# askerlee/segtran

Measured on AMD Instinct MI355X. Metric: train-step images/sec (cfg2, re-associated op order), higher is better.
Workload: dtype f32; 1 GPU; REFUGE fundus 2D, segtran eff-b4, translayers 3, layercompress 1,1,2,2, 512x512, bs 6/GPU; global_batch=6, per_gpu_batch=6, parallelism=dp1, step=fwd+BCE/Dice+bwd+allreduce+clip+BertAdam, op_order=re-associated, ranks=1

## Files before the change

### include/segx.h

```cpp
#ifndef SEGX_H
#define SEGX_H
#include <stdint.h>
#ifdef __cplusplus
extern "C" {
#endif

int segx_version(void);
int segx_last_error(char* buf, int buflen);

enum { SEGX_EPI_NONE = 0, SEGX_EPI_GELU = 1 ,
       SEGX_EPI_SWISH = 2 ,
       SEGX_EPI_RELU = 3  };
enum { SEGX_BIAS_NONE = 0, SEGX_BIAS_N = 1 , SEGX_BIAS_M = 2  };
enum { SEGX_ENGINE_F32 = 0, SEGX_ENGINE_BF16X6 = 1 };
enum { SEGX_ENGINE_SEL_DEFAULT = 0, SEGX_ENGINE_SEL_F32 = 1, SEGX_ENGINE_SEL_BF16X6 = 2 };
enum { SEGX_TILE_AUTO = 0, SEGX_TILE_128x128 = 1, SEGX_TILE_64x64 = 2, SEGX_TILE_128x32 = 3, SEGX_TILE_32x128 = 4, SEGX_TILE_64x128 = 5,
       SEGX_TILE_256x128 = 6, SEGX_TILE_WS128x128 = 7, SEGX_TILE_WS128x256 = 8, SEGX_TILE_WS64x256 = 9,
       SEGX_TILE_WS96x256 = 10, SEGX_TILE_WS256x96 = 11,
       SEGX_TILE_SKINNY_NT = 12   };
typedef struct {
    int32_t M, N, K, nb0, nb1;
    int64_t a_b0, a_b1, a_m, a_k;
    int64_t b_b0, b_b1, b_n, b_k;
    int64_t c_b0, c_b1, c_m;
// ... 102 lines not shown
int segx_team_status(int clear);
int segx_team_cap(void);
int segx_occupy(int wgs, int heavy, float ms, float* sink, void* stream);
int segx_bn_act_bwd2(const float* dY, const float* X, const float* mean, const float* var, const float* w, const float* b,
                     float* dX, float* dw, float* db, float* ws, int B, int C, int64_t S, float eps, int act, int training,
                     const float* gate, const float* dpool, float inv_S, float dc_p, uint64_t seed, uint64_t offset, int64_t dy_bs, int64_t ws_floats, void* stream);
int segx_se_fwd2(const float* psum, int nch, float inv_S, const float* W1, const float* b1, const float* W2, const float* b2, const float* Wproj,
                 float* p, float* hpre, float* gate, float* Wb, int B, int C, int Cs, int M, void* stream);
int64_t segx_se_ws2_floats(int B, int C, int Cs);
int segx_se_bwd2(const float* dWb, const float* Wproj, const float* dgate, const float* gate, const float* hpre, const float* p, const float* W1,
                 const float* W2, float inv_S, float* dpool, float* dW1, float* db1, float* dW2, float* db2, float* dWproj, float* ws,
                 int B, int C, int Cs, int M, void* stream);
int segx_dwconv2d_fwd(const float* X, const float* W, float* Y, int B, int C, int H, int Wd, int OH, int OW, int k, int stride,
                      int pad_t, int pad_l, void* stream);
int64_t segx_dwconv2d_pool_chunks(int OH, int OW);
int segx_dwconv2d_bias_act_pool(const float* X, const float* W, const float* bias, float* Y, float* psum, int B, int C, int H, int Wd, int OH, int OW,
                                int k, int stride, int pad_t, int pad_l, int act, void* stream);
int segx_dwconv2d_bwd_data(const float* dY, const float* W, float* dX, int B, int C, int H, int Wd, int OH, int OW, int k,
                           int stride, int pad_t, int pad_l, void* stream);
int64_t segx_dwconv2d_wgrad_rows(int OH, int OW);
int64_t segx_dwconv2d_bwd_fused_rows(int H, int Wd, int OH, int OW, int k, int stride, int pad_t, int pad_l);
int segx_dwconv2d_bwd_fused(const float* dY, const float* X, const float* W, float* dX, float* part, int B, int C, int H, int Wd, int OH, int OW,
                            int k, int stride, int pad_t, int pad_l, void* stream);
int segx_dwconv2d_bwd_weight_direct(const float* dY, const float* X, float* dW, int B, int C, int H, int Wd, int OH, int OW, int k,
                                    int stride, int pad_t, int pad_l, void* stream);
int segx_dwconv2d_bwd_weight(const float* dY, const float* X, float* part, int B, int C, int H, int Wd, int OH, int OW, int k,
                             int stride, int pad_t, int pad_l, void* stream);
int segx_plane_scale(const float* X, const float* gate, float* Y, int64_t planes, int64_t S, void* stream);
int segx_plane_bias_add(const float* X, const float* bias, float* Y, int64_t planes, int C, int64_t S, void* stream);
int segx_plane_dot(const float* A, const float* Bm, float* out, int64_t planes, int64_t S, void* stream);

int64_t segx_gn_ws_floats(int B, int C, int G);
int segx_groupnorm_fwd(const float* X, const float* w, const float* b, float* Y, float* mean, float* rstd, float* ws,
                       int B, int C, int G, int64_t S, float eps, void* stream);
int segx_groupnorm_bwd(const float* dY, const float* X, const float* w, const float* mean, const float* rstd, float* dX,
                       float* dw, float* db, float* ws, int B, int C, int G, int64_t S, float* plane_dx_sums, void* stream);
int64_t segx_interp_gn_nparts(int64_t float4_per_plane, int cpg);
int segx_interp_linear_fwd_axis2_gn(const float* in, const float* base, float* out, int64_t outer, int n1_in, int n1_out, int n2_in, int n2_out,
                                    int64_t inner, int cpg, float* parts, int nparts, void* stream);
int segx_groupnorm_fwd_parts(const float* X, const float* parts, int nparts, const float* w, const float* b, float* Y, float* mean, float* rstd,
                             int B, int C, int G, int64_t S, float eps, void* stream);
int segx_groupnorm_stats_parts(const float* parts, int nparts, float* mean, float* rstd, int BG, float eps, void* stream);
int segx_gn_fold_bwd_proj(const float* dOut, const float* Wb, int NC, const float* X, const float* mean, const float* rstd, const float* A, const float* Bc,
                          float* dX, float* plane_sums, float* ws, int B, int C, int G, int64_t S, void* stream);
int segx_gn_fold_bwd(const float* Gd, const float* X, const float* mean, const float* rstd, const float* A, const float* Bc, float* dX, float* plane_sums,
                     float* ws, int B, int C, int G, int64_t S, void* stream);
// ... 130 lines not shown
```

### segtran_amd/csrc/backbone.hip

```cpp
#include "common.h"
#include <mutex>
#include <unordered_map>

namespace segx {

enum { ACT_NONE = 0, ACT_SWISH = 1, ACT_RELU = 2, ACT_LEAKY = 3  };

__device__ __forceinline__ float sigm(float x) { return 1.0f / (1.0f + __expf(-x)); }
__device__ __forceinline__ float act_fwd(float u, int act) {
    return act == ACT_SWISH ? u * sigm(u) : act == ACT_RELU ? fmaxf(u, 0.f) : act == ACT_LEAKY ? (u > 0.f ? u : 0.2f * u) : u;
}
__device__ __forceinline__ float act_grad(float u, int act) {
    if (act == ACT_SWISH) { const float s = sigm(u); return s * (1.0f + u * (1.0f - s)); }
    if (act == ACT_RELU) return u > 0.f ? 1.0f : 0.f;
    if (act == ACT_LEAKY) return u > 0.f ? 1.0f : 0.2f;
    return 1.0f;
}

__device__ __forceinline__ float drop_connect_scale(float p, uint64_t seed, uint64_t offset, const uint64_t* __restrict__ rbase, int sample) {
    if (!(p > 0.f)) return 1.0f;
    return dropout_scale(seed, 0, offset + (rbase ? *rbase : 0) + (uint64_t)sample, p, 1.0f / (1.0f - p));
}
__device__ __forceinline__ void bn_fold_sums(const float* __restrict__ ws, int c, int nparts, float& a, float& q) {
    const int lane = threadIdx.x & 63;
    const float2* p = reinterpret_cast<const float2*>(ws) + (int64_t)c * nparts;
    a = 0.f; q = 0.f;
    for (int i = lane; i < nparts; i += 64) { const float2 v = p[i]; a += v.x; q += v.y; }
    a = wave_sum(a); q = wave_sum(q);
}

constexpr int BN_SLABS = 8;
static inline int bn_slabs(int64_t S) { const int64_t n = S / 8192; return (int)(n < 1 ? 1 : n > BN_SLABS ? BN_SLABS : n); }

__global__ __launch_bounds__(256) void bn_act_bwd_stage1(const float* __restrict__ dY, const float* __restrict__ X, const float* __restrict__ mean,
                                                         const float* __restrict__ var, const float* __restrict__ w, const float* __restrict__ b,
                                                         float* __restrict__ ws, int C, int64_t S, float eps, int act,
                                                         const float* __restrict__ gate, const float* __restrict__ dpool, float inv_S,
                                                         float dc_p, uint64_t seed, uint64_t offset, const uint64_t* __restrict__ rbase, int64_t dy_bs) {
    __shared__ float red[4];
    const int c = blockIdx.x, bb = blockIdx.y, slab = blockIdx.z;
// ... 1742 lines not shown
```

### segtran_amd/csrc/common.h

```cpp
#pragma once
#include <hip/hip_runtime.h>
#include <stdint.h>
#include <stdio.h>
#include <stdarg.h>
#include <string.h>
#include <math.h>
#include <atomic>
#include "../../include/segx.h"

typedef float f32x16 __attribute__((ext_vector_type(16)));
typedef float f32x4 __attribute__((ext_vector_type(4)));

namespace segx {

inline char* err_buf() { static thread_local char buf[512] = {0}; return buf; }
inline int fail(int code, const char* fmt, ...) {
    va_list ap; va_start(ap, fmt); vsnprintf(err_buf(), 512, fmt, ap); va_end(ap); return code;
}
inline int check_launch(const char* what) {
    hipError_t e = hipGetLastError();
    if (e != hipSuccess) return fail((int)e, "%s: %s", what, hipGetErrorString(e));
    return 0;
}
#ifndef SEGX_MIN_WAVES_PER_SIMD
// ... 115 lines not shown
    return v;
}
template <int NW> __device__ __forceinline__ float block_sum(float v, float* red) {
    v = wave_sum(v);
    const int lane = threadIdx.x & 63, w = threadIdx.x >> 6;
    __syncthreads();
    if (lane == 0) red[w] = v;
    __syncthreads();
    float s = 0.f;
#pragma unroll
    for (int i = 0; i < NW; ++i) s += red[i];
    return s;
}
template <int NW> __device__ __forceinline__ float block_max(float v, float* red) {
    v = wave_max(v);
    const int lane = threadIdx.x & 63, w = threadIdx.x >> 6;
    __syncthreads();
    if (lane == 0) red[w] = v;
    __syncthreads();
    float s = red[0];
#pragma unroll
    for (int i = 1; i < NW; ++i) s = fmaxf(s, red[i]);
    return s;
}

struct u32x4 { unsigned x, y, z, w; };
__device__ __forceinline__ u32x4 philox4(uint64_t seed, uint64_t ctr) {
    unsigned c0 = (unsigned)ctr, c1 = (unsigned)(ctr >> 32), c2 = 0x5eed5eedu, c3 = 0u;
    unsigned k0 = (unsigned)seed, k1 = (unsigned)(seed >> 32);
#pragma unroll
    for (int r = 0; r < 7; ++r) {
        const unsigned h0 = __umulhi(0xD2511F53u, c0), l0 = 0xD2511F53u * c0;
        const unsigned h1 = __umulhi(0xCD9E8D57u, c2), l1 = 0xCD9E8D57u * c2;
        const unsigned n0 = h1 ^ c1 ^ k0, n2 = h0 ^ c3 ^ k1;
        c0 = n0; c1 = l1; c2 = n2; c3 = l0;
        k0 += 0x9E3779B9u; k1 += 0xBB67AE85u;
    }
    u32x4 o; o.x = c0; o.y = c1; o.z = c2; o.w = c3; return o;
}
__device__ __forceinline__ float keep_of(unsigned u, float p, float inv_keep) {
    return ((float)(u >> 8) * (1.0f / 16777216.0f) >= p) ? inv_keep : 0.0f;
}
__device__ __forceinline__ float4 dropout_scale4(uint64_t seed, uint64_t offset, uint64_t idx0, float p, float inv_keep) {
    const u32x4 r = philox4(seed, (offset + idx0) >> 2);
    return make_float4(keep_of(r.x, p, inv_keep), keep_of(r.y, p, inv_keep), keep_of(r.z, p, inv_keep), keep_of(r.w, p, inv_keep));
}
// ... 82 lines not shown
```

### segtran_amd/efficientnet/model.py

```python
import math
import torch
from torch import nn
from torch.nn import functional as F

from .. import functional as SF

BN_MOM, BN_EPS = 1 - 0.99, 1e-3

_BASE = [(1, 3, 1, 1, 32, 16, 0.25), (2, 3, 2, 6, 16, 24, 0.25), (2, 5, 2, 6, 24, 40, 0.25), (3, 3, 2, 6, 40, 80, 0.25),
         (3, 5, 1, 6, 80, 112, 0.25), (4, 5, 2, 6, 112, 192, 0.25), (1, 3, 1, 6, 192, 320, 0.25)]
_PARAMS = {'efficientnet-b0': (1.0, 1.0, 224, 0.2), 'efficientnet-b1': (1.0, 1.1, 240, 0.2),
           'efficientnet-b2': (1.1, 1.2, 260, 0.3), 'efficientnet-b3': (1.2, 1.4, 300, 0.3),
           'efficientnet-b4': (1.4, 1.8, 380, 0.4), 'efficientnet-b5': (1.6, 2.2, 456, 0.4),
           'efficientnet-b6': (1.8, 2.6, 528, 0.5), 'efficientnet-b7': (2.0, 3.1, 600, 0.5)}


def round_filters(filters, width, divisor=8):
    filters *= width
    new = max(divisor, int(filters + divisor / 2) // divisor * divisor)
    if new < 0.9 * filters:
        new += divisor
    return int(new)


# ... 40 lines not shown
        s = bn.weight.double() / torch.sqrt(bn.running_var.double() + bn.eps)
        w = (weight.double() * s.view(-1, *([1] * (weight.dim() - 1)))).float().contiguous()
        b = (bn.bias.double() - bn.running_mean.double() * s).float().contiguous()
    return w, b


class MBConvBlock(nn.Module):
    def __init__(self, k, s, e, cin, cout, se_ratio, image_size):
        super().__init__()
        self.stride, self.expand_ratio, self.input_filters, self.output_filters = s, e, cin, cout
        oup = cin * e
        if e != 1:
            self._expand_conv = Conv2dStaticSamePadding(cin, oup, 1, image_size=image_size, bias=False)
            self._bn0 = nn.BatchNorm2d(oup, momentum=BN_MOM, eps=BN_EPS)
        self._depthwise_conv = Conv2dStaticSamePadding(oup, oup, k, stride=s, image_size=image_size, groups=oup, bias=False)
        self._bn1 = nn.BatchNorm2d(oup, momentum=BN_MOM, eps=BN_EPS)
        nsq = max(1, int(cin * se_ratio))
        self._se_reduce = Conv2dStaticSamePadding(oup, nsq, 1, image_size=1)
        self._se_expand = Conv2dStaticSamePadding(nsq, oup, 1, image_size=1)
        self._project_conv = Conv2dStaticSamePadding(oup, cout, 1, image_size=math.ceil(image_size / s), bias=False)
        self._bn2 = nn.BatchNorm2d(cout, momentum=BN_MOM, eps=BN_EPS)

    gate_in_weights = True

    def folded_operands(self):
        f0 = fold_conv_bn(self._expand_conv.weight, self._bn0) if self.expand_ratio != 1 else None
        return f0, fold_conv_bn(self._depthwise_conv.weight, self._bn1), fold_conv_bn(self._project_conv.weight, self._bn2)

    def forward_folded(self, inputs, folded):
        f0, (w1, b1), (w2, b2) = folded
        x = inputs
        skip = self.stride == 1 and self.input_filters == self.output_filters
        if f0 is not None:
            x = SF.conv1x1(x, f0[0], f0[1], act=SF.ACT_SWISH)
        dw = self._depthwise_conv
        y, psum, nch = SF.dwconv2d_bias_act_pool(x, w1, b1, dw.stride[0], dw.static_pad, SF.ACT_SWISH)
        Wb = SF.se_gate_weights(y, psum, nch, self._se_reduce.weight, self._se_reduce.bias, self._se_expand.weight, self._se_expand.bias, w2)
        return SF.conv1x1_per_sample_bias(y, Wb, b2, resid=inputs if skip else None)

    def forward(self, inputs, drop_connect_rate=None):
        x = skip_in = inputs
        skip = self.stride == 1 and self.input_filters == self.output_filters
        if self.expand_ratio != 1:
            x = SF.bn_act(self._expand_conv(x), self._bn0, SF.ACT_SWISH)
        se = (self._se_reduce.weight, self._se_reduce.bias, self._se_expand.weight, self._se_expand.bias)
        rate = float(drop_connect_rate) if (skip and drop_connect_rate and self.training) else 0.0
        if MBConvBlock.gate_in_weights:
            y, Wb = SF.bn_act_gate_weights(self._depthwise_conv(x), self._bn1, SF.ACT_SWISH, *se, self._project_conv.weight)
            x = SF.conv1x1_per_sample(y, Wb)
        else:
            x = self._project_conv(SF.bn_act_se(self._depthwise_conv(x), self._bn1, SF.ACT_SWISH, *se))
        return SF.bn_act(x, self._bn2, SF.ACT_NONE, resid=skip_in if skip else None, drop_connect=rate)


class EfficientNet(nn.Module):
    def __init__(self, model_name='efficientnet-b4', stem_stride=2, drop_connect_rate=0.2, num_classes=1000):
        super().__init__()
        width, depth, res, _ = _PARAMS[model_name]
        self.drop_connect_rate = drop_connect_rate
        self.stem_stride = stem_stride
        c0 = round_filters(32, width)
        self._conv_stem = Conv2dStaticSamePadding(3, c0, 3, stride=stem_stride, image_size=res, bias=False)
        self._bn0 = nn.BatchNorm2d(c0, momentum=BN_MOM, eps=BN_EPS)
        size = math.ceil(res / 2)
        self._blocks = nn.ModuleList([])
        self.endpoint_seg_indices = [0, 1, 2, 4]
        self.endpoint_blk_indices = []
        for i, (r, k, s, e, cin, cout, se) in enumerate(_BASE):
            cin, cout, r = round_filters(cin, width), round_filters(cout, width), round_repeats(r, depth)
            self._blocks.append(MBConvBlock(k, s, e, cin, cout, se, size))
# ... 127 lines not shown
```

### segtran_amd/functional.py

```python
import math
import torch
import torch.nn.functional as F
from . import segx
from .segx import EPI_NONE, EPI_GELU, EPI_SWISH, EPI_RELU, BIAS_NONE, BIAS_N, BIAS_M

LN_EPS = 1e-12


_MRO = torch.autograd.Function.__mro__
_fast_apply = torch._C._FunctionBase in _MRO and not any('apply' in c.__dict__ for c in _MRO[1:_MRO.index(torch._C._FunctionBase)])


class _Fn(torch.autograd.Function):

    @classmethod
    def apply(cls, *args):
        if _fast_apply and not torch._C._are_functorch_transforms_active():
            return super(torch.autograd.Function, cls).apply(*args)
        return super().apply(*args)


def _live(t):
    return t.requires_grad and torch.is_grad_enabled()

# ... 974 lines not shown
        ctx.cfg = (B, C, S, eps, act, training, n)
        ctx.shapes = (tuple(w1.shape), tuple(w2.shape), tuple(Wproj.shape))
        ctx.save_for_backward(x, mean, var, w, b, p, hpre, gate, W1, W2, Wp)
        return y, Wb

    @staticmethod
    def backward(ctx, dy, dWb):
        L = segx.lib()
        x, mean, var, w, b, p, hpre, gate, W1, W2, Wp = ctx.saved_tensors
        S = ctx.cfg[2]
        w1s, w2s, wps = ctx.shapes
        dWb = _c(dWb) if dWb is not None else torch.zeros(gate.shape[0], Wp.shape[0], Wp.shape[1], dtype=torch.float32, device=x.device)
        dpool, dW1, db1, dW2, db2, dWp = _se_excite_backward(L, x, dWb, Wp, None, gate, hpre, p, W1, W2, S)
        dx, dw, db = _bn_act_backward(L, _c(dy), x, mean, var, w, b, ctx.cfg, None, dpool, 1.0)
        return dx, dw, db, None, None, None, None, None, None, dW1.view(w1s), db1, dW2.view(w2s), db2, dWp.view(wps)


def bn_act_gate_weights(x, bn, act, w1, b1, w2, b2, proj_weight):
    _bn_tick(bn)
    return _BNActGateW.apply(x, bn.weight, bn.bias, bn.running_mean, bn.running_var, bn.training, float(bn.momentum), float(bn.eps), act, w1, b1, w2, b2,
                             proj_weight)


def conv1x1_per_sample(x, Wb, bias=None):
    B, Cin = x.shape[0], x.shape[1]
    S = x.numel() // (B * Cin)
    Cout = Wb.shape[1]
    if bias is None:
        spec = GemmSpec(Cout, S, Cin, (Cout * Cin, 0, Cin, 1), (Cin * S, 0, 1, S), (Cout * S, 0, S), (B, Cout) + tuple(x.shape[2:]), nb=(B, 1))
        return bgemm(Wb, x, spec)
    spec = GemmSpec(Cout, S, Cin, (Cout * Cin, 0, Cin, 1), (Cin * S, 0, 1, S), (Cout * S, 0, S), (B, Cout) + tuple(x.shape[2:]), nb=(B, 1), bias_mode=BIAS_M, bias_b0=Cout)
    return bgemm(Wb, x, spec, bias=_c(bias))


def dwconv2d_bias_act_pool(x, w, bias, stride, pad, act=ACT_SWISH, pool=True):
    if act not in (ACT_NONE, ACT_SWISH):
        raise NotImplementedError('dwconv2d_bias_act_pool: act is ACT_NONE or ACT_SWISH')
    _no_grad_operands('dwconv2d_bias_act_pool', x, w, bias)
    L = segx.lib()
    x, w = _c(x), _c(w)
    B, C, H, W = x.shape
    k, stride = w.shape[-1], int(stride)
    pl, pr, pt, pb = (int(v) for v in pad)
    OH, OW = (H + pt + pb - k) // stride + 1, (W + pl + pr - k) // stride + 1
    y = _empty(x, B, C, OH, OW)
    nch = L.dwconv2d_pool_chunks(OH, OW) if pool else 0
# ... 1225 lines not shown
```

### segtran_amd/segx.py

```python
import contextlib
import ctypes
import enum
import os
import torch

_HERE = os.path.dirname(os.path.abspath(__file__))
LIB_PATH = os.path.join(_HERE, 'lib', 'libsegx.so')

c_f = ctypes.c_float
c_i = ctypes.c_int32
c_l = ctypes.c_int64
c_u = ctypes.c_uint64
c_p = ctypes.c_void_p


class GemmDesc(ctypes.Structure):
    _fields_ = [('M', c_i), ('N', c_i), ('K', c_i), ('nb0', c_i), ('nb1', c_i),
                ('a_b0', c_l), ('a_b1', c_l), ('a_m', c_l), ('a_k', c_l),
                ('b_b0', c_l), ('b_b1', c_l), ('b_n', c_l), ('b_k', c_l),
                ('c_b0', c_l), ('c_b1', c_l), ('c_m', c_l),
                ('alpha', c_f), ('epilogue', c_i), ('bias_mode', c_i), ('bias_b1', c_l),
                ('bias', c_p), ('aux', c_p), ('gmax', c_p),
                ('dropout_p', c_f), ('seed', c_u), ('offset', c_u),
                ('splitk', c_i), ('workspace', c_p), ('tile', c_i), ('bias_b0', c_l), ('batch_reduce', c_i), ('engine', c_i),
# ... 325 lines not shown
            self._chk_t(Y)
            assert Y.device == X.device and Y.dtype == torch.float32 and Y.stride(1) == S and Y.stride(0) == y_bs and Y[0].is_contiguous()
            Y = Y.data_ptr()
        self._call('segx_bn_act_fwd2', X, X, parts, nparts, mean, var, run_mean, run_var, momentum, w, b, Y, psum, resid, float(dc_p), seed, offset, B, C, S, eps, act,
                   0 if parts is None else parts.numel(), int(y_bs))

    def bn_act_bwd2(self, dY, X, mean, var, w, b, dX, dw, db, ws, B, C, S, eps, act, training, gate=None, dpool=None, inv_S=0.0, dc_p=0.0, seed=0, offset=0, dy_bs=0):
        self._chk_t(dY, X, mean, var, w, b, dX, dw, db, ws, gate, dpool)
        for t in (X, mean, var, w, b, dX, dw, db, ws):
            assert t.is_contiguous()
        assert dy_bs or dY.is_contiguous()
        rc = self.c.segx_bn_act_bwd2(_ptr(dY), _ptr(X), _ptr(mean), _ptr(var), _ptr(w), _ptr(b), _ptr(dX), _ptr(dw), _ptr(db), _ptr(ws), B, C, S, eps, act, training,
                                     _ptr(gate), _ptr(dpool), float(inv_S), float(dc_p), seed, offset, int(dy_bs), ws.numel(), self.stream(X))
        self.check(rc, 'segx_bn_act_bwd2')

    def se_fwd2(self, psum, nch, inv_S, W1, b1, W2, b2, Wproj, p, hpre, gate, Wb, B, C, Cs, M):
        self._call('segx_se_fwd2', gate, psum, nch, inv_S, W1, b1, W2, b2, Wproj, p, hpre, gate, Wb, B, C, Cs, M)

    def se_ws2(self, B, C, Cs):
        return int(self.c.segx_se_ws2_floats(B, C, Cs))

    def se_bwd2(self, dWb, Wproj, dgate, gate, hpre, p, W1, W2, inv_S, dpool, dW1, db1, dW2, db2, dWproj, ws, B, C, Cs, M):
        self._call('segx_se_bwd2', gate, dWb, Wproj, dgate, gate, hpre, p, W1, W2, inv_S, dpool, dW1, db1, dW2, db2, dWproj, ws, B, C, Cs, M)

    def dwconv2d_fwd(self, X, W, Y, B, C, H, Wd, OH, OW, k, stride, pt, pl):
        self._call('segx_dwconv2d_fwd', X, X, W, Y, B, C, H, Wd, OH, OW, k, stride, pt, pl)

    def dwconv2d_pool_chunks(self, OH, OW):
        return int(self.c.segx_dwconv2d_pool_chunks(OH, OW))

    def dwconv2d_bias_act_pool(self, X, W, bias, Y, psum, B, C, H, Wd, OH, OW, k, stride, pt, pl, act):
        self._call('segx_dwconv2d_bias_act_pool', X, X, W, bias, Y, psum, B, C, H, Wd, OH, OW, k, stride, pt, pl, act)

    def dwconv2d_bwd_data(self, dY, W, dX, B, C, H, Wd, OH, OW, k, stride, pt, pl):
        self._call('segx_dwconv2d_bwd_data', dY, dY, W, dX, B, C, H, Wd, OH, OW, k, stride, pt, pl)

    def dwconv2d_bwd_weight_direct(self, dY, X, dW, B, C, H, Wd, OH, OW, k, stride, pt, pl):
        self._chk_t(dY, X, dW)
        rc = self.c.segx_dwconv2d_bwd_weight_direct(_ptr(dY), _ptr(X), _ptr(dW), B, C, H, Wd, OH, OW, k, stride, pt, pl, self.stream(X))
        if rc < 0:
            self.check(rc, 'segx_dwconv2d_bwd_weight_direct')
        return rc == 1

    def dwconv2d_bwd_fused_rows(self, H, W, OH, OW, k, stride, pad_t, pad_l):
        return int(self.c.segx_dwconv2d_bwd_fused_rows(H, W, OH, OW, k, stride, pad_t, pad_l))

# ... 346 lines not shown
    'segx_mt_bertadam_step': 'pppppppppppiiifffddfpp', 'segx_mt_gather': 'pppppiiip',
    'segx_gn_ws_floats': 'iii', 'segx_groupnorm_fwd': 'pppppppiiilfp', 'segx_groupnorm_bwd': 'pppppppppiiilpp',
    'segx_interp_gn_nparts': 'li', 'segx_interp_linear_fwd_axis2_gn': 'pppliiiilipip', 'segx_groupnorm_fwd_parts': 'ppipppppiiilfp',
    'segx_groupnorm_stats_parts': 'pippifp', 'segx_gn_fold_bwd': 'pppppppppiiilp', 'segx_bridge_mask': 'ppppiiiiiiiiip', 'segx_gn_fold_bwd_proj': 'ppippppppppiiilp',
    'segx_interp_linear_fwd': 'pppliiiiiip', 'segx_interp_linear_fwd_axis2': 'pppliiiilp', 'segx_interp_linear_bwd_axis2': 'ppliiiilp', 'segx_interp_linear_bwd': 'ppliiiiiip', 'segx_interp_linear_bwd_axis': 'ppliilfp',
    'segx_axis_gather': 'pplpp', 'segx_pixel_shuffle2': 'ppliiip', 'segx_add_noise': 'ppplffiuup', 'segx_resize2d': 'ppliiiiiip', 'segx_color_blend': 'ppilippip',
    'segx_gray_mean_ws_floats': 'il', 'segx_gray_mean': 'pppilip', 'segx_normalize': 'ppiilfppp',
    'segx_x6_presplit_elems': 'iiii', 'segx_x6_presplit': 'piilliillpp',
    'segx_tune': 'ii', 'segx_tune_get': 'i', 'segx_x3_launches': '', 'segx_gemm_route': 'pppp', 'segx_set_rng_base': 'p', 'segx_rng_advance': 'pup', 'segx_resized_crop3d': 'pplpp', 'segx_stem_compose_fwd': 'ppppiiiiip', 'segx_stem_compose_bwd': 'pppppppiiiiip', 'segx_bridge_input': 'ppiiiiiip', 'segx_stem_s2d_input': 'ppiiiiiip', 'segx_conv2d_stem_fwd': 'pppiiiiiiiiiiip', 'segx_conv2d_stem_im2col': 'ppiiiiiiiiiiip', 'segx_dropout': 'pplfuup', 'segx_avgpool2_fwd': 'ppliip', 'segx_avgpool2_bwd': 'ppliip', 'segx_transpose': 'ppliip', 'segx_interp_linear_fwd_axis': 'pppliilfp', 'segx_window_accum': 'pppiipp', 'segx_harden_segmap': 'ppppiilifp', 'segx_window_gather': 'ppppiiipp', 'segx_window_merge': 'pppppiiipifp', 'segx_dice_ws_floats': 'll', 'segx_dice_sums': 'pppllp',
    'segx_surface_border': 'ppliiiip', 'segx_edt_sq': 'ppliiip', 'segx_surface_hist': 'pppliiiip',
    'segx_ccl2d': 'pippliip', 'segx_frag_keep2': 'ppliip', 'segx_frag_apply': 'ppppliiip', 'segx_row_extent': 'ppliifp', 'segx_nhot_to_values': 'ppplilp',
    'segx_conv3d_fwd': 'pppiipipp', 'segx_conv3d_fwd_packed': 'pppiipipp', 'segx_conv3d_fwd_packed_bs': 'pppiipipllp', 'segx_conv3d_bwd_weight_packed_bs': 'pppiipipllp', 'segx_conv3d_pack_weights': 'ppiiiip', 'segx_conv3d_splitk': 'iipi', 'segx_conv3d_route': 'iipiiiip', 'segx_conv3d_fwd_terms': 'iipiii', 'segx_conv3d_flip_weights': 'ppiiip', 'segx_conv3d_bwd_weight': 'pppiipipp', 'segx_conv3d_bwd_weight_packed': 'pppiipipp', 'segx_conv3d_unpack_wgrad': 'ppiiip',
    'segx_conv3d_halo_ok': 'iip', 'segx_conv3d_halo_wq_floats': 'ii', 'segx_conv3d_halo_pack': 'ppiiip', 'segx_conv3d_halo_fwd': 'pppiipllip', 'segx_conv3d_halo_bias_act_fwd': 'ppppiiplliip', 'segx_conv3d_fwd_bias_act': 'ppppiipipillip', 'segx_bias_map_relu': 'ppilp', 'segx_conv3d_halo_wgrad_ok': 'iip', 'segx_conv3d_halo_wgrad_ws_floats': 'iip', 'segx_conv3d_halo_wgrad': 'ppppiipllp',
    'segx_conv3d_bwd_data_direct': 'ppppiipp', 'segx_nonzero_mask': 'ppiiiiiiiip', 'segx_label_nhot': 'ppiilip',
    'segx_maxpool3d_fwd': 'ppplpp', 'segx_maxpool3d_bwd': 'ppplppp',
    'segx_bn_ws_floats': 'iil', 
    'segx_dwconv2d_fwd': 'pppiiiiiiiiiip', 'segx_dwconv2d_bwd_data': 'pppiiiiiiiiiip',
    'segx_dwconv2d_pool_chunks': 'ii', 'segx_dwconv2d_bias_act_pool': 'pppppiiiiiiiiiiip', 'segx_conv2d_stem_bias_act_fwd': 'ppppiiiiiiiiiiiip',
    'segx_dwconv2d_bwd_weight': 'pppiiiiiiiiiip', 'segx_dwconv2d_bwd_weight_direct': 'pppiiiiiiiiiip', 'segx_dwconv2d_wgrad_rows': 'ii', 'segx_dwconv2d_bwd_fused_rows': 'iiiiiiii', 'segx_dwconv2d_bwd_fused': 'pppppiiiiiiiiiip', 'segx_plane_scale': 'pppllp', 'segx_plane_dot': 'pppllp',
     'segx_plane_bias_add': 'ppplilp', 
    'segx_plane_chunks': 'l', 'segx_bn_pool_chunks': 'ili', 'segx_bn_parts_floats': 'iil', 'segx_bn_stats_local': 'pppiilp',
    'segx_bn_act_fwd2': 'ppippppfpppppfuuiilfillp', 'segx_bn_act_bwd2': 'ppppppppppiilfiippffuullp',
    'segx_team_status': 'i', 'segx_team_cap': '', 'segx_occupy': 'iifpp',
    'segx_se_fwd2': 'pifpppppppppiiiip', 'segx_se_ws2_floats': 'iii', 'segx_se_bwd2': 'ppppppppfpppppppiiiip',
    'segx_bn_act_bwd_reduce': 'pppppppppiilfippffuup', 'segx_bn_act_bwd_apply': 'pppppppppiilfifppffuup',
}

_LIB = None
DEFAULT_ENGINE = 'x6'


def lib():
    global _LIB
    if _LIB is None:
        _LIB = SegxLib(LIB_PATH)
        _LIB.set_engine(os.environ.get('SEGX_ENGINE', DEFAULT_ENGINE))
    return _LIB


def use_library(libobj):
    global _LIB
    _LIB = libobj
```

Baseline: 98.48 images/s.

## Fuse MBConv middle BN0-swish, depthwise conv, BN1-swish and pooling into one kernel

Adds an mbconv_mid kernel pair that keeps a whole channel plane for all samples on chip. The forward pass computes BN0 statistics, applies swish, runs the depthwise conv through LDS, computes BN1 statistics, applies swish and produces the SE pooled sums in a single launch. The backward pass fuses the BN1 backward, depthwise data and weight gradients, and the BN0 backward. The aim is to remove several full-tensor HBM round trips and kernel launches per MBConv block, at the cost of one block per channel, heavy register/LDS use, and shape restrictions that only the served small spatial sizes take.

```diff
diff --git a/include/segx.h b/include/segx.h
--- a/include/segx.h
+++ b/include/segx.h
@@ -148,6 +148,14 @@
 int64_t segx_dwconv2d_bwd_fused_rows(int H, int Wd, int OH, int OW, int k, int stride, int pad_t, int pad_l);
 int segx_dwconv2d_bwd_fused(const float* dY, const float* X, const float* W, float* dX, float* part, int B, int C, int H, int Wd, int OH, int OW,
                             int k, int stride, int pad_t, int pad_l, void* stream);
+int segx_mbconv_mid_ok(int B, int C, int H, int W, int k);
+int segx_mbconv_mid_fwd(const float* E, const float* w0, const float* b0, float* run_mean0, float* run_var0, const float* Wdw, const float* w1, const float* b1,
+                        float* run_mean1, float* run_var1, float* D, float* Y, float* psum, float* mean0, float* var0, float* mean1, float* var1,
+                        float momentum0, float eps0, float momentum1, float eps1, int B, int C, int H, int W, int k, void* stream);
+int segx_mbconv_mid_bwd(const float* dY, const float* dpool, const float* D, const float* E, const float* mean0, const float* var0, const float* mean1,
+                        const float* var1, const float* w0, const float* b0, const float* w1, const float* b1, const float* Wdw,
+                        float* dE, float* dw0, float* db0, float* dw1, float* db1, float* dWdw, float inv_S, float eps0, float eps1,
+                        int B, int C, int H, int W, int k, void* stream);
 int segx_dwconv2d_bwd_weight_direct(const float* dY, const float* X, float* dW, int B, int C, int H, int Wd, int OH, int OW, int k,
                                     int stride, int pad_t, int pad_l, void* stream);
 int segx_dwconv2d_bwd_weight(const float* dY, const float* X, float* part, int B, int C, int H, int Wd, int OH, int OW, int k,
diff --git a/segtran_amd/csrc/backbone.hip b/segtran_amd/csrc/backbone.hip
--- a/segtran_amd/csrc/backbone.hip
+++ b/segtran_amd/csrc/backbone.hip
@@ -4,18 +4,6 @@
 
 namespace segx {
 
-enum { ACT_NONE = 0, ACT_SWISH = 1, ACT_RELU = 2, ACT_LEAKY = 3  };
-
-__device__ __forceinline__ float sigm(float x) { return 1.0f / (1.0f + __expf(-x)); }
-__device__ __forceinline__ float act_fwd(float u, int act) {
-    return act == ACT_SWISH ? u * sigm(u) : act == ACT_RELU ? fmaxf(u, 0.f) : act == ACT_LEAKY ? (u > 0.f ? u : 0.2f * u) : u;
-}
-__device__ __forceinline__ float act_grad(float u, int act) {
-    if (act == ACT_SWISH) { const float s = sigm(u); return s * (1.0f + u * (1.0f - s)); }
-    if (act == ACT_RELU) return u > 0.f ? 1.0f : 0.f;
-    if (act == ACT_LEAKY) return u > 0.f ? 1.0f : 0.2f;
-    return 1.0f;
-}
 
 __device__ __forceinline__ float drop_connect_scale(float p, uint64_t seed, uint64_t offset, const uint64_t* __restrict__ rbase, int sample) {
     if (!(p > 0.f)) return 1.0f;
diff --git a/segtran_amd/csrc/common.h b/segtran_amd/csrc/common.h
--- a/segtran_amd/csrc/common.h
+++ b/segtran_amd/csrc/common.h
@@ -161,6 +161,19 @@
 #pragma unroll
     for (int i = 1; i < NW; ++i) s = fmaxf(s, red[i]);
     return s;
+}
+
+enum { ACT_NONE = 0, ACT_SWISH = 1, ACT_RELU = 2, ACT_LEAKY = 3  };
+
+__device__ __forceinline__ float sigm(float x) { return 1.0f / (1.0f + __expf(-x)); }
+__device__ __forceinline__ float act_fwd(float u, int act) {
+    return act == ACT_SWISH ? u * sigm(u) : act == ACT_RELU ? fmaxf(u, 0.f) : act == ACT_LEAKY ? (u > 0.f ? u : 0.2f * u) : u;
+}
+__device__ __forceinline__ float act_grad(float u, int act) {
+    if (act == ACT_SWISH) { const float s = sigm(u); return s * (1.0f + u * (1.0f - s)); }
+    if (act == ACT_RELU) return u > 0.f ? 1.0f : 0.f;
+    if (act == ACT_LEAKY) return u > 0.f ? 1.0f : 0.2f;
+    return 1.0f;
 }
 
 struct u32x4 { unsigned x, y, z, w; };
diff --git a/segtran_amd/csrc/mbconv_mid.hip b/segtran_amd/csrc/mbconv_mid.hip
--- /dev/null
+++ b/segtran_amd/csrc/mbconv_mid.hip
@@ -0,0 +1,342 @@
+#include "common.h"
+#include <initializer_list>
+
+namespace segx {
+
+constexpr int MID_BMAX = 6;
+
+template <int NT> __device__ __forceinline__ void mid_guards(f32x4* pl, int H, int W4) {
+    for (int r = threadIdx.x; r <= H; r += NT) pl[r * (W4 + 1)] = f32x4{0.f, 0.f, 0.f, 0.f};
+}
+__device__ __forceinline__ void mid_window(float (&e)[12], const f32x4* pl, int p, int r, int dr, int H, int W4) {
+    const bool rok = (unsigned)(r + dr) < (unsigned)H;
+    const f32x4* q = pl + (rok ? p + dr * (W4 + 1) : p);
+    const f32x4 a = q[-1], m = q[0], z = q[1];
+    e[0] = rok ? a.x : 0.f; e[1] = rok ? a.y : 0.f; e[2] = rok ? a.z : 0.f; e[3] = rok ? a.w : 0.f;
+    e[4] = rok ? m.x : 0.f; e[5] = rok ? m.y : 0.f; e[6] = rok ? m.z : 0.f; e[7] = rok ? m.w : 0.f;
+    e[8] = rok ? z.x : 0.f; e[9] = rok ? z.y : 0.f; e[10] = rok ? z.z : 0.f; e[11] = rok ? z.w : 0.f;
+}
+template <int NW, int KP>
+__device__ __forceinline__ void mid_stats(f32x4 (&v)[MID_BMAX][KP], int B, float n, float* red, float& m, float& q) {
+    float s = 0.f;
+#pragma unroll
+    for (int b = 0; b < MID_BMAX; ++b)
+#pragma unroll
+        for (int k = 0; k < KP; ++k) {
+            if (b >= B) v[b][k] = f32x4{0.f, 0.f, 0.f, 0.f};
+            s += (v[b][k].x + v[b][k].y) + (v[b][k].z + v[b][k].w);
+        }
+    m = block_sum<NW>(s, red) / n;
+    q = 0.f;
+#pragma unroll
+    for (int b = 0; b < MID_BMAX; ++b)
+#pragma unroll
+        for (int k = 0; k < KP; ++k) {
+            const float d0 = v[b][k].x - m, d1 = v[b][k].y - m, d2 = v[b][k].z - m, d3 = v[b][k].w - m;
+            q += b < B ? (d0 * d0 + d1 * d1) + (d2 * d2 + d3 * d3) : 0.f;
+        }
+    q = block_sum<NW>(q, red);
+}
+__device__ __forceinline__ void mid_running(float* run_mean, float* run_var, int c, float momentum, float m, float q, float n) {
+    if (run_mean) {
+        run_mean[c] = (1.0f - momentum) * run_mean[c] + momentum * m;
+        run_var[c] = (1.0f - momentum) * run_var[c] + momentum * (q / fmaxf(n - 1.0f, 1.0f));
+    }
+}
+
+struct MidFwdArgs {
+    const float* E; const float* w0; const float* b0; float* rm0; float* rv0; const float* Wdw; const float* w1; const float* b1; float* rm1; float* rv1;
+    float* D; float* Y; float* psum; float* mean0; float* var0; float* mean1; float* var1;
+    float mom0, eps0, mom1, eps1; int C, H, W4;
+};
+template <int KP, int K>
+__global__ __launch_bounds__(256) SEGX_MIN_WAVES_PER_SIMD(KP == 1 ? 4 : 2) void mbconv_mid_fwd_kernel(MidFwdArgs g, int B) {
+    constexpr int NT = 256, P = K / 2, S4 = NT * KP;
+    __shared__ float red[4];
+    __shared__ f32x4 plane[2 * S4 + 1];
+    const int tl = threadIdx.x, c = blockIdx.x, C = g.C, H = g.H, W4 = g.W4;
+    constexpr int64_t S = 4 * S4;
+    unsigned off[KP]; int row[KP], pos[KP];
+#pragma unroll
+    for (int k = 0; k < KP; ++k) { const int j = tl + NT * k; off[k] = 16u * (unsigned)j; row[k] = j / W4; pos[k] = j + row[k] + 1; }
+    mid_guards<NT>(plane, H, W4);
+    f32x4 v[MID_BMAX][KP];
+#pragma unroll
+    for (int b = 0; b < MID_BMAX; ++b) {
+        const ws_gptr xb = ws_uniform_base(g.E + ((int64_t)(b < B ? b : 0) * C + c) * S);
+#pragma unroll
+        for (int k = 0; k < KP; ++k) v[b][k] = ws_load<f32x4>(xb, off[k]);
+    }
+    __builtin_amdgcn_sched_barrier(0);
+    float w[K * K];
+#pragma unroll
+    for (int i = 0; i < K * K; ++i) w[i] = g.Wdw[(int64_t)c * K * K + i];
+    const float n = (float)B * (float)S;
+    float m, q;
+    mid_stats<4, KP>(v, B, n, red, m, q);
+    float var = q / n;
+    if (tl == 0) { g.mean0[c] = m; g.var0[c] = var; mid_running(g.rm0, g.rv0, c, g.mom0, m, q, n); }
+    const float sc0 = rsqrtf(var + g.eps0) * g.w0[c], sh0 = g.b0[c] - m * sc0;
+#pragma unroll
+    for (int b = 0; b < MID_BMAX; ++b) {
+        if (b >= B) break;
+#pragma unroll
+        for (int k = 0; k < KP; ++k) {
+            f32x4 o;
+            o.x = act_fwd(v[b][k].x * sc0 + sh0, ACT_SWISH); o.y = act_fwd(v[b][k].y * sc0 + sh0, ACT_SWISH);
+            o.z = act_fwd(v[b][k].z * sc0 + sh0, ACT_SWISH); o.w = act_fwd(v[b][k].w * sc0 + sh0, ACT_SWISH);
+            plane[pos[k]] = o;
+        }
+        __syncthreads();
+        const ws_gptr_w db = ws_uniform_base_w(g.D + ((int64_t)b * C + c) * S);
+#pragma unroll
+        for (int k = 0; k < KP; ++k) {
+            float acc[4] = {0.f, 0.f, 0.f, 0.f};
+#pragma unroll
+            for (int ky = 0; ky < K; ++ky) {
+                float e[12];
+                mid_window(e, plane, pos[k], row[k], ky - P, H, W4);
+#pragma unroll
+                for (int j = 0; j < 4; ++j)
+#pragma unroll
+                    for (int kx = 0; kx < K; ++kx) acc[j] += w[ky * K + kx] * e[4 + j + kx - P];
+#pragma unroll
+                for (int j = 0; j < 4; ++j) SEGX_PIN(acc[j]);
+            }
+            v[b][k] = f32x4{acc[0], acc[1], acc[2], acc[3]};
+            ws_store<f32x4>(db, off[k], v[b][k]);
+        }
+        __syncthreads();
+        __builtin_amdgcn_sched_barrier(0);
+    }
+    mid_stats<4, KP>(v, B, n, red, m, q);
+    var = q / n;
+    if (tl == 0) { g.mean1[c] = m; g.var1[c] = var; mid_running(g.rm1, g.rv1, c, g.mom1, m, q, n); }
+    const float sc1 = rsqrtf(var + g.eps1) * g.w1[c], sh1 = g.b1[c] - m * sc1;
+#pragma unroll
+    for (int b = 0; b < MID_BMAX; ++b) {
+        if (b >= B) break;
+        const ws_gptr_w yb = ws_uniform_base_w(g.Y + ((int64_t)b * C + c) * S);
+        float acc = 0.f;
+#pragma unroll
+        for (int k = 0; k < KP; ++k) {
+            f32x4 o;
+            o.x = act_fwd(v[b][k].x * sc1 + sh1, ACT_SWISH); o.y = act_fwd(v[b][k].y * sc1 + sh1, ACT_SWISH);
+            o.z = act_fwd(v[b][k].z * sc1 + sh1, ACT_SWISH); o.w = act_fwd(v[b][k].w * sc1 + sh1, ACT_SWISH);
+            ws_store<f32x4>(yb, off[k], o);
+            acc += (o.x + o.y) + (o.z + o.w);
+        }
+        acc = block_sum<4>(acc, red);
+        if (tl == 0) g.psum[(int64_t)b * C + c] = acc;
+        __builtin_amdgcn_sched_barrier(0);
+    }
+}
+
+__device__ __forceinline__ double wave_sum_d(double v) {
+#pragma unroll
+    for (int o = 32; o > 0; o >>= 1) v += __shfl_xor(v, o);
+    return v;
+}
+template <int NW> __device__ __forceinline__ double block_sum_d(double v, double* red) {
+    v = wave_sum_d(v);
+    __syncthreads();
+    if ((threadIdx.x & 63) == 0) red[threadIdx.x >> 6] = v;
+    __syncthreads();
+    double s = 0.0;
+#pragma unroll
+    for (int i = 0; i < NW; ++i) s += red[i];
+    return s;
+}
+
+struct MidBwdArgs {
+    const float* dY; const float* dpool; const float* D; const float* E;
+    const float* mean0; const float* var0; const float* mean1; const float* var1;
+    const float* w0; const float* b0; const float* w1; const float* b1; const float* Wdw;
+    float* dE; float* dw0; float* db0; float* dw1; float* db1; float* dWdw;
+    float inv_S, eps0, eps1; int C, H, W4;
+};
+template <int NT, int KP, int K, bool HL>
+__global__ __launch_bounds__(NT) void mbconv_mid_bwd_kernel(MidBwdArgs g, int B) {
+    constexpr int NW = NT / 64, P = K / 2, S4 = NT * KP, KK = K * K;
+    __shared__ double red[NW];
+    __shared__ double wred[NW][KK];
+    __shared__ f32x4 plane[2 * S4 + 1];
+    __shared__ f32x4 hl[HL ? MID_BMAX * S4 : 1];
+    const int tl = threadIdx.x, c = blockIdx.x, C = g.C, H = g.H, W4 = g.W4;
+    constexpr int64_t S = 4 * S4;
+    unsigned off[KP]; int row[KP], pos[KP];
+#pragma unroll
+    for (int k = 0; k < KP; ++k) { const int j = tl + NT * k; off[k] = 16u * (unsigned)j; row[k] = j / W4; pos[k] = j + row[k] + 1; }
+    mid_guards<NT>(plane, H, W4);
+    f32x4 h[MID_BMAX][KP], d[MID_BMAX][KP];
+    auto hget = [&](int b, int k) -> f32x4 { if constexpr (HL) return hl[(b * KP + k) * NT + tl]; else return h[b][k]; };
+    auto hput = [&](int b, int k, f32x4 x) { if constexpr (HL) hl[(b * KP + k) * NT + tl] = x; else h[b][k] = x; };
+#pragma unroll
+    for (int b = 0; b < MID_BMAX; ++b) {
+        const int64_t po = ((int64_t)(b < B ? b : 0) * C + c) * S;
+        const ws_gptr xb = ws_uniform_base(g.D + po), gb = ws_uniform_base(g.dY + po);
+#pragma unroll
+        for (int k = 0; k < KP; ++k) { h[b][k] = ws_load<f32x4>(xb, off[k]); d[b][k] = ws_load<f32x4>(gb, off[k]); }
+    }
+    f32x4 ev[KP];
+    {
+        const ws_gptr eb = ws_uniform_base(g.E + (int64_t)c * S);
+#pragma unroll
+        for (int k = 0; k < KP; ++k) ev[k] = ws_load<f32x4>(eb, off[k]);
+    }
+    __builtin_amdgcn_sched_barrier(0);
+    float w[KK], dwa[KK];
+#pragma unroll
+    for (int i = 0; i < KK; ++i) { w[i] = g.Wdw[(int64_t)c * KK + i]; dwa[i] = 0.f; }
+    const double inv_n = 1.0 / ((double)B * (double)S);
+    const float rstd1 = rsqrtf(g.var1[c] + g.eps1), m1 = g.mean1[c], w1c = g.w1[c], b1c = g.b1[c];
+    double a = 0.0, q = 0.0;
+#pragma unroll
+    for (int b = 0; b < MID_BMAX; ++b) {
+        const bool bok = b < B;
+        const float dp = g.dpool[(bok ? b : 0) * C + c] * g.inv_S;
+#pragma unroll
+        for (int k = 0; k < KP; ++k) {
+            const f32x4 xv = h[b][k], gv = d[b][k];
+            f32x4 hh, dd;
+            hh.x = (xv.x - m1) * rstd1; hh.y = (xv.y - m1) * rstd1; hh.z = (xv.z - m1) * rstd1; hh.w = (xv.w - m1) * rstd1;
+            dd.x = (gv.x + dp) * act_grad(hh.x * w1c + b1c, ACT_SWISH); dd.y = (gv.y + dp) * act_grad(hh.y * w1c + b1c, ACT_SWISH);
+            dd.z = (gv.z + dp) * act_grad(hh.z * w1c + b1c, ACT_SWISH); dd.w = (gv.w + dp) * act_grad(hh.w * w1c + b1c, ACT_SWISH);
+            if (!bok) { dd = f32x4{0.f, 0.f, 0.f, 0.f}; hh = dd; }
+            hput(b, k, hh); d[b][k] = dd;
+            a += (double)((dd.x + dd.y) + (dd.z + dd.w)); q += (double)((dd.x * hh.x + dd.y * hh.y) + (dd.z * hh.z + dd.w * hh.w));
+        }
+        __builtin_amdgcn_sched_barrier(0);
+    }
+    a = block_sum_d<NW>(a, red); q = block_sum_d<NW>(q, red);
+    if (tl == 0) { g.db1[c] = (float)a; g.dw1[c] = (float)q; }
+    const double k1 = a * inv_n, k2 = q * inv_n, sc1 = (double)(w1c * rstd1);
+    const float k1f = (float)k1, k2f = (float)k2, sc1f = w1c * rstd1;
+    const float rstd0 = rsqrtf(g.var0[c] + g.eps0), m0 = g.mean0[c], sc0 = rstd0 * g.w0[c], sh0 = g.b0[c] - m0 * sc0;
+    double a0 = 0.0, q0 = 0.0;
+#pragma unroll
+    for (int b = 0; b < MID_BMAX; ++b) {
+        if (b >= B) break;
+#pragma unroll
+        for (int k = 0; k < KP; ++k) {
+            const f32x4 hh = hget(b, k);
+            f32x4 o;
+            if constexpr (HL) {
+                o.x = (float)(sc1 * ((double)d[b][k].x - k1 - (double)hh.x * k2)); o.y = (float)(sc1 * ((double)d[b][k].y - k1 - (double)hh.y * k2));
+                o.z = (float)(sc1 * ((double)d[b][k].z - k1 - (double)hh.z * k2)); o.w = (float)(sc1 * ((double)d[b][k].w - k1 - (double)hh.w * k2));
+            } else {
+                o.x = sc1f * (d[b][k].x - k1f - hh.x * k2f); o.y = sc1f * (d[b][k].y - k1f - hh.y * k2f);
+                o.z = sc1f * (d[b][k].z - k1f - hh.z * k2f); o.w = sc1f * (d[b][k].w - k1f - hh.w * k2f);
+            }
+            plane[pos[k]] = o;
+        }
+        __syncthreads();
+#pragma unroll
+        for (int k = 0; k < KP; ++k) {
+            const f32x4 xv = ev[k];
+            const float u[4] = {xv.x * sc0 + sh0, xv.y * sc0 + sh0, xv.z * sc0 + sh0, xv.w * sc0 + sh0};
+            float ep[4], de[4] = {0.f, 0.f, 0.f, 0.f};
+#pragma unroll
+            for (int i = 0; i < 4; ++i) ep[i] = act_fwd(u[i], ACT_SWISH);
+#pragma unroll
+            for (int ry = -P; ry <= P; ++ry) {
+                float e[12];
+                mid_window(e, plane, pos[k], row[k], ry, H, W4);
+#pragma unroll
+                for (int rx = -P; rx <= P; ++rx) {
+                    const int t = (P - ry) * K + (P - rx);
+#pragma unroll
+                    for (int i = 0; i < 4; ++i) {
+                        de[i] = __builtin_fmaf(w[t], e[4 + i + rx], de[i]); dwa[t] = __builtin_fmaf(ep[i], e[4 + i + rx], dwa[t]);
+                        SEGX_PIN(de[i]); SEGX_PIN(dwa[t]);
+                    }
+                }
+                __builtin_amdgcn_sched_barrier(0);
+            }
+            f32x4 hh, dd;
+            hh.x = (xv.x - m0) * rstd0; hh.y = (xv.y - m0) * rstd0; hh.z = (xv.z - m0) * rstd0; hh.w = (xv.w - m0) * rstd0;
+            dd.x = de[0] * act_grad(u[0], ACT_SWISH); dd.y = de[1] * act_grad(u[1], ACT_SWISH);
+            dd.z = de[2] * act_grad(u[2], ACT_SWISH); dd.w = de[3] * act_grad(u[3], ACT_SWISH);
+            hput(b, k, hh); d[b][k] = dd;
+            a0 += (double)((dd.x + dd.y) + (dd.z + dd.w)); q0 += (double)((dd.x * hh.x + dd.y * hh.y) + (dd.z * hh.z + dd.w * hh.w));
+        }
+        if (b + 1 < MID_BMAX) {
+            const ws_gptr eb = ws_uniform_base(g.E + ((int64_t)(b + 1 < B ? b + 1 : b) * C + c) * S);
+#pragma unroll
+            for (int k = 0; k < KP; ++k) ev[k] = ws_load<f32x4>(eb, off[k]);
+        }
+        __syncthreads();
+        __builtin_amdgcn_sched_barrier(0);
+    }
+    a0 = block_sum_d<NW>(a0, red); q0 = block_sum_d<NW>(q0, red);
+    if (tl == 0) { g.db0[c] = (float)a0; g.dw0[c] = (float)q0; }
+    const float j1 = (float)(a0 * inv_n), j2 = (float)(q0 * inv_n);
+#pragma unroll
+    for (int b = 0; b < MID_BMAX; ++b) {
+        if (b >= B) break;
+        const ws_gptr_w ob = ws_uniform_base_w(g.dE + ((int64_t)b * C + c) * S);
+#pragma unroll
+        for (int k = 0; k < KP; ++k) {
+            const f32x4 hh = hget(b, k);
+            f32x4 o;
+            o.x = sc0 * (d[b][k].x - j1 - hh.x * j2); o.y = sc0 * (d[b][k].y - j1 - hh.y * j2);
+            o.z = sc0 * (d[b][k].z - j1 - hh.z * j2); o.w = sc0 * (d[b][k].w - j1 - hh.w * j2);
+            ws_store<f32x4>(ob, off[k], o);
+        }
+        __builtin_amdgcn_sched_barrier(0);
+    }
+#pragma unroll
+    for (int i = 0; i < KK; ++i) { const double s = wave_sum_d((double)dwa[i]); if ((tl & 63) == 0) wred[tl >> 6][i] = s; }
+    __syncthreads();
+    if (tl < KK) {
+        double s = 0.0;
+#pragma unroll
+        for (int i = 0; i < NW; ++i) s += wred[i][tl];
+        g.dWdw[(int64_t)c * KK + tl] = (float)s;
+    }
+}
+
+static inline bool mid_serves(int B, int C, int H, int W, int k) {
+    return B >= 1 && B <= MID_BMAX && C >= 1 && H >= 1 && W >= 4 && W % 4 == 0 && (k == 3 || k == 5) && ((int64_t)H * W == 1024 || (int64_t)H * W == 4096);
+}
+static inline bool mid_aligned(std::initializer_list<const void*> ps) {
+    for (const void* p : ps) if (reinterpret_cast<uintptr_t>(p) & 15) return false;
+    return true;
+}
+
+}
+
+using namespace segx;
+#define SEGX_STREAM hipStream_t stream = (hipStream_t)stream_
+
+extern "C" int segx_mbconv_mid_ok(int B, int C, int H, int W, int k) { return mid_serves(B, C, H, W, k) ? 1 : 0; }
+
+extern "C" int segx_mbconv_mid_fwd(const float* E, const float* w0, const float* b0, float* run_mean0, float* run_var0, const float* Wdw, const float* w1, const float* b1,
+                                   float* run_mean1, float* run_var1, float* D, float* Y, float* psum, float* mean0, float* var0, float* mean1, float* var1,
+                                   float momentum0, float eps0, float momentum1, float eps1, int B, int C, int H, int W, int k, void* stream_) {
+    SEGX_STREAM; SEGX_REQUIRE(E && w0 && b0 && Wdw && w1 && b1 && D && Y && psum && mean0 && var0 && mean1 && var1 && (!run_mean0 == !run_var0) && (!run_mean1 == !run_var1),
+                              "segx_mbconv_mid_fwd: bad args");
+    SEGX_REQUIRE(mid_serves(B, C, H, W, k), "segx_mbconv_mid_fwd: shape not served (segx_mbconv_mid_ok == 0)");
+    SEGX_REQUIRE(mid_aligned({E, D, Y}), "segx_mbconv_mid_fwd: tensors must be 16-byte aligned");
+    const MidFwdArgs g{E, w0, b0, run_mean0, run_var0, Wdw, w1, b1, run_mean1, run_var1, D, Y, psum, mean0, var0, mean1, var1, momentum0, eps0, momentum1, eps1, C, H, W / 4};
+#define SEGX_MID_F(KP, K) hipLaunchKernelGGL((mbconv_mid_fwd_kernel<KP, K>), dim3((unsigned)C), dim3(256), 0, stream, g, B)
+    if (H * W == 4096) { if (k == 3) SEGX_MID_F(4, 3); else SEGX_MID_F(4, 5); }
+    else { if (k == 3) SEGX_MID_F(1, 3); else SEGX_MID_F(1, 5); }
+#undef SEGX_MID_F
+    return check_launch("segx_mbconv_mid_fwd");
+}
+
+extern "C" int segx_mbconv_mid_bwd(const float* dY, const float* dpool, const float* D, const float* E, const float* mean0, const float* var0, const float* mean1,
+                                   const float* var1, const float* w0, const float* b0, const float* w1, const float* b1, const float* Wdw,
+                                   float* dE, float* dw0, float* db0, float* dw1, float* db1, float* dWdw, float inv_S, float eps0, float eps1,
+                                   int B, int C, int H, int W, int k, void* stream_) {
+    SEGX_STREAM; SEGX_REQUIRE(dY && dpool && D && E && mean0 && var0 && mean1 && var1 && w0 && b0 && w1 && b1 && Wdw && dE && dw0 && db0 && dw1 && db1 && dWdw, "segx_mbconv_mid_bwd: bad args");
+    SEGX_REQUIRE(mid_serves(B, C, H, W, k), "segx_mbconv_mid_bwd: shape not served (segx_mbconv_mid_ok == 0)");
+    SEGX_REQUIRE(mid_aligned({dY, D, E, dE}), "segx_mbconv_mid_bwd: tensors must be 16-byte aligned");
+    const MidBwdArgs g{dY, dpool, D, E, mean0, var0, mean1, var1, w0, b0, w1, b1, Wdw, dE, dw0, db0, dw1, db1, dWdw, inv_S, eps0, eps1, C, H, W / 4};
+#define SEGX_MID_B(NT, KP, K, HL) hipLaunchKernelGGL((mbconv_mid_bwd_kernel<NT, KP, K, HL>), dim3((unsigned)C), dim3(NT), 0, stream, g, B)
+    if (H * W == 4096) { if (k == 3) SEGX_MID_B(1024, 1, 3, true); else SEGX_MID_B(512, 2, 5, true); }
+    else { if (k == 3) SEGX_MID_B(256, 1, 3, false); else SEGX_MID_B(256, 1, 5, false); }
+#undef SEGX_MID_B
+    return check_launch("segx_mbconv_mid_bwd");
+}
diff --git a/segtran_amd/efficientnet/model.py b/segtran_amd/efficientnet/model.py
--- a/segtran_amd/efficientnet/model.py
+++ b/segtran_amd/efficientnet/model.py
@@ -86,6 +86,16 @@
         self._bn2 = nn.BatchNorm2d(cout, momentum=BN_MOM, eps=BN_EPS)
 
     gate_in_weights = True
+    fused_middle = True
+
+    def _takes_fused_middle(self, x):
+        if not (MBConvBlock.fused_middle and MBConvBlock.gate_in_weights and self.training and SF._bn_stats_sync is None and self.expand_ratio != 1):
+            return False
+        dw = self._depthwise_conv
+        k = dw.kernel_size[0]
+        if not (self._bn0.training and self._bn1.training and dw.stride == (1, 1) and dw.kernel_size == (k, k) and tuple(dw.static_pad) == (k // 2,) * 4):
+            return False
+        return x.dim() == 4 and x.dtype == torch.float32 and SF.mbconv_mid_ok((x.shape[0], dw.in_channels, x.shape[2], x.shape[3]), k)
 
     def folded_operands(self):
         f0 = fold_conv_bn(self._expand_conv.weight, self._bn0) if self.expand_ratio != 1 else None
@@ -105,11 +115,15 @@
     def forward(self, inputs, drop_connect_rate=None):
         x = skip_in = inputs
         skip = self.stride == 1 and self.input_filters == self.output_filters
-        if self.expand_ratio != 1:
+        fused = self._takes_fused_middle(x)
+        if self.expand_ratio != 1 and not fused:
             x = SF.bn_act(self._expand_conv(x), self._bn0, SF.ACT_SWISH)
         se = (self._se_reduce.weight, self._se_reduce.bias, self._se_expand.weight, self._se_expand.bias)
         rate = float(drop_connect_rate) if (skip and drop_connect_rate and self.training) else 0.0
-        if MBConvBlock.gate_in_weights:
+        if fused:
+            y, Wb = SF.mbconv_mid(self._expand_conv(x), self._bn0, self._depthwise_conv.weight, self._bn1, *se, self._project_conv.weight)
+            x = SF.conv1x1_per_sample(y, Wb)
+        elif MBConvBlock.gate_in_weights:
             y, Wb = SF.bn_act_gate_weights(self._depthwise_conv(x), self._bn1, SF.ACT_SWISH, *se, self._project_conv.weight)
             x = SF.conv1x1_per_sample(y, Wb)
         else:
diff --git a/segtran_amd/functional.py b/segtran_amd/functional.py
--- a/segtran_amd/functional.py
+++ b/segtran_amd/functional.py
@@ -1020,6 +1020,54 @@
                              proj_weight)
 
 
+class _MBConvMid(_Fn):
+
+    @staticmethod
+    def forward(ctx, e, w0, b0, rm0, rv0, mom0, eps0, wdw, w1, b1, rm1, rv1, mom1, eps1, sw1, sb1, sw2, sb2, Wproj):
+        L = segx.lib()
+        e, wdw = _c(e), _c(wdw)
+        if e.data_ptr() % 16:
+            e = e.clone()
+        B, C, H, W = e.shape
+        k, S = wdw.shape[-1], H * W
+        Wp = _c(Wproj.reshape(Wproj.shape[0], C))
+        d, y = torch.empty_like(e), torch.empty_like(e)
+        psum, stats = _empty(e, B * C), _empty(e, 4, C)
+        L.mbconv_mid_fwd(e, w0, b0, rm0, rv0, wdw, w1, b1, rm1, rv1, d, y, psum, stats[0], stats[1], stats[2], stats[3], mom0, eps0, mom1, eps1, B, C, H, W, k)
+        p, hpre, gate, W1, W2, Wb = _se_excite(L, y, psum, 1, S, sw1, sb1, sw2, sb2, Wp)
+        ctx.cfg = (B, C, H, W, k, eps0, eps1)
+        ctx.shapes = (tuple(sw1.shape), tuple(sw2.shape), tuple(Wproj.shape), tuple(wdw.shape))
+        ctx.save_for_backward(e, d, stats, w0, b0, wdw, w1, b1, p, hpre, gate, W1, W2, Wp)
+        return y, Wb
+
+    @staticmethod
+    def backward(ctx, dy, dWb):
+        L = segx.lib()
+        e, d, stats, w0, b0, wdw, w1, b1, p, hpre, gate, W1, W2, Wp = ctx.saved_tensors
+        B, C, H, W, k, eps0, eps1 = ctx.cfg
+        w1s, w2s, wps, wds = ctx.shapes
+        dWb = _c(dWb) if dWb is not None else torch.zeros(B, Wp.shape[0], C, dtype=torch.float32, device=e.device)
+        dy = _c(dy) if dy is not None else torch.zeros_like(e)
+        if dy.data_ptr() % 16:
+            dy = dy.clone()
+        dpool, dW1, db1, dW2, db2, dWp = _se_excite_backward(L, e, dWb, Wp, None, gate, hpre, p, W1, W2, H * W)
+        de, g, dwd = torch.empty_like(e), _empty(e, 4, C), _empty(e, C * k * k)
+        L.mbconv_mid_bwd(dy, dpool, d, e, stats[0], stats[1], stats[2], stats[3], w0, b0, w1, b1, wdw, de, g[0], g[1], g[2], g[3], dwd, 1.0, eps0, eps1, B, C, H, W, k)
+        return (de, g[0], g[1], None, None, None, None, dwd.view(wds), g[2], g[3], None, None, None, None,
+                dW1.view(w1s), db1, dW2.view(w2s), db2, dWp.view(wps))
+
+
+def mbconv_mid_ok(e_shape, k):
+    return len(e_shape) == 4 and segx.lib().mbconv_mid_ok(e_shape[0], e_shape[1], e_shape[2], e_shape[3], int(k))
+
+
+def mbconv_mid(e, bn0, dw_weight, bn1, w1, b1, w2, b2, proj_weight):
+    _bn_tick(bn0)
+    _bn_tick(bn1)
+    return _MBConvMid.apply(e, bn0.weight, bn0.bias, bn0.running_mean, bn0.running_var, float(bn0.momentum), float(bn0.eps), dw_weight,
+                            bn1.weight, bn1.bias, bn1.running_mean, bn1.running_var, float(bn1.momentum), float(bn1.eps), w1, b1, w2, b2, proj_weight)
+
+
 def conv1x1_per_sample(x, Wb, bias=None):
     B, Cin = x.shape[0], x.shape[1]
     S = x.numel() // (B * Cin)
diff --git a/segtran_amd/segx.py b/segtran_amd/segx.py
--- a/segtran_amd/segx.py
+++ b/segtran_amd/segx.py
@@ -371,6 +371,17 @@
 
     def se_bwd2(self, dWb, Wproj, dgate, gate, hpre, p, W1, W2, inv_S, dpool, dW1, db1, dW2, db2, dWproj, ws, B, C, Cs, M):
         self._call('segx_se_bwd2', gate, dWb, Wproj, dgate, gate, hpre, p, W1, W2, inv_S, dpool, dW1, db1, dW2, db2, dWproj, ws, B, C, Cs, M)
+
+    def mbconv_mid_ok(self, B, C, H, W, k):
+        return bool(self.c.segx_mbconv_mid_ok(B, C, H, W, k))
+
+    def mbconv_mid_fwd(self, E, w0, b0, rm0, rv0, Wdw, w1, b1, rm1, rv1, D, Y, psum, mean0, var0, mean1, var1, mom0, eps0, mom1, eps1, B, C, H, W, k):
+        self._call('segx_mbconv_mid_fwd', E, E, w0, b0, rm0, rv0, Wdw, w1, b1, rm1, rv1, D, Y, psum, mean0, var0, mean1, var1, float(mom0), float(eps0), float(mom1), float(eps1),
+                   B, C, H, W, k)
+
+    def mbconv_mid_bwd(self, dY, dpool, D, E, mean0, var0, mean1, var1, w0, b0, w1, b1, Wdw, dE, dw0, db0, dw1, db1, dWdw, inv_S, eps0, eps1, B, C, H, W, k):
+        self._call('segx_mbconv_mid_bwd', dY, dY, dpool, D, E, mean0, var0, mean1, var1, w0, b0, w1, b1, Wdw, dE, dw0, db0, dw1, db1, dWdw, float(inv_S), float(eps0), float(eps1),
+                   B, C, H, W, k)
 
     def dwconv2d_fwd(self, X, W, Y, B, C, H, Wd, OH, OW, k, stride, pt, pl):
         self._call('segx_dwconv2d_fwd', X, X, W, Y, B, C, H, Wd, OH, OW, k, stride, pt, pl)
@@ -763,6 +774,7 @@
     'segx_plane_chunks': 'l', 'segx_bn_pool_chunks': 'ili', 'segx_bn_parts_floats': 'iil', 'segx_bn_stats_local': 'pppiilp',
     'segx_bn_act_fwd2': 'ppippppfpppppfuuiilfillp', 'segx_bn_act_bwd2': 'ppppppppppiilfiippffuullp',
     'segx_team_status': 'i', 'segx_team_cap': '', 'segx_occupy': 'iifpp',
+    'segx_mbconv_mid_ok': 'iiiii', 'segx_mbconv_mid_fwd': 'p' * 17 + 'ffff' + 'iiiii' + 'p', 'segx_mbconv_mid_bwd': 'p' * 19 + 'fff' + 'iiiii' + 'p',
     'segx_se_fwd2': 'pifpppppppppiiiip', 'segx_se_ws2_floats': 'iii', 'segx_se_bwd2': 'ppppppppfpppppppiiiip',
     'segx_bn_act_bwd_reduce': 'pppppppppiilfippffuup', 'segx_bn_act_bwd_apply': 'pppppppppiilfifppffuup',
 }
```

After: 100.9 images/s (median of 6 runs). 2.4% higher.
